# cchao0116/EasyDGL

Hardware: AMD Instinct MI355X
Metric: sequences/sec (fwd+bwd+Adam) B=512 L=100 d=128 |I|=20K (higher is better)
Workload: dtype bf16

## Files before the change

### easydgl_amd/csrc/k_encode.hip

```cpp
#include "edgl_common.h"
#include "batch_prep.h"
#include "red_batch.h"
#include "encode_scatter.h"

namespace {

using namespace enc_scatter;

struct EncP {
    const int64_t* ids; const float* ts; const void* item_tab; const float* pos_tab; const float* mark_emb;
    const uint8_t* mark_table; const float* tscale;
    int B, T, C, E, I; int64_t mask_id; float time_scale;
    float rate; const uint64_t* rng; uint32_t stream_id;
    void* x0; float* spans; uint8_t* marks;
    int dhp, dht; float sq;
};

template <typename T>
__device__ __forceinline__ void encode_fwd_block(const EncP& p, long block) {
    const int cpr = p.C >> 3;
    const long gid = block * blockDim.x + threadIdx.x;
    const long row = gid / cpr;
    if (row >= (long)p.B * p.T) return;
    const int cv = (int)(gid % cpr), c0 = cv * 8, j0 = c0 >> 1;
// ... 179 lines not shown
    __shared__ int s_lead[SROWS];
    const int SR = p.srows;
    const long rows = (long)p.B * p.T, r0 = (long)blockIdx.x * SR;
    const int tid = threadIdx.x;
    if (tid < SR) s_id[tid] = (r0 + tid < rows) ? (int)p.ids[r0 + tid] : 0;
    if (tid >= SR && tid < SROWS) s_id[tid] = -1;
    const int cpr = p.C / 4, rows_par = 256 / cpr;
    const int cv = tid % cpr, rl = tid / cpr, c0 = cv * 4;
    constexpr int MAXR = 16;
    Frag4<T> g[MAXR];
    const bool worker = tid < rows_par * cpr;
    auto item_grad = [&](long row) {
        Frag4<T> v = frag_ld<T>(reinterpret_cast<const T*>(p.dx0) + row * 3 * p.C + c0);
        if (p.add1) {
            const Frag4<T> a = frag_ld<T>(reinterpret_cast<const T*>(p.add1) + row * p.C + c0);
            const Frag4<T> b = frag_ld<T>(reinterpret_cast<const T*>(p.add2) + row * p.C + c0);
#pragma unroll
            for (int j = 0; j < 4; ++j) v.v[j] = from_f32<T>(to_f32(v.v[j]) + to_f32(a.v[j]) + to_f32(b.v[j]));
        }
        return v;
    };
#pragma unroll
    for (int k = 0; k < MAXR; ++k) g[k] = item_grad(min(r0 + rl + (long)k * rows_par, rows - 1));
    for (int i = tid; i < SR * p.C; i += 256) acc[i] = 0.f;
    __syncthreads();
    if (tid < SR) {
        const int id = s_id[tid];
        int lead = tid;
        for (int j4 = (tid >> 2); j4 >= 0; --j4) {
            const int4 v = *reinterpret_cast<const int4*>(s_id + 4 * j4);
            const int j = 4 * j4;
            if (v.w == id && j + 3 < tid) lead = j + 3;
            if (v.z == id && j + 2 < tid) lead = j + 2;
            if (v.y == id && j + 1 < tid) lead = j + 1;
            if (v.x == id && j < tid) lead = j;
        }
        s_lead[tid] = lead;
    }
    __syncthreads();
    const DropKey dk = make_dropkey(p.rng, p.stream_id, p.rate);
    const float sq = p.sq;
    if (worker) {
#pragma unroll
        for (int k = 0; k < MAXR; ++k) {
            const int r = rl + k * rows_par;
            if (r >= SR || s_id[r] == 0) continue;
            const long row = r0 + r;
            float* dst = acc + s_lead[r] * p.C + c0;
            float gv[4];
#pragma unroll
            for (int j = 0; j < 4; ++j) gv[j] = to_f32(g[k].v[j]);
            drop_apply4(dk, (uint64_t)row * 3 * p.C + c0, gv);
#pragma unroll
            for (int j = 0; j < 4; ++j) atomicAdd(dst + j, sq * gv[j]);
        }
        for (int r = rl + MAXR * rows_par; r < SR; r += rows_par) {
            if (s_id[r] == 0) continue;
            const long row = r0 + r;
            const Frag4<T> g0 = item_grad(row);
            float* dst = acc + s_lead[r] * p.C + c0;
            float gv[4];
#pragma unroll
            for (int j = 0; j < 4; ++j) gv[j] = to_f32(g0.v[j]);
            drop_apply4(dk, (uint64_t)row * 3 * p.C + c0, gv);
#pragma unroll
            for (int j = 0; j < 4; ++j) atomicAdd(dst + j, sq * gv[j]);
        }
    }
    __syncthreads();
    for (int i = tid; i < SR * p.C; i += 256) {
        const int r = i / p.C, c = i % p.C;
        if (s_lead[r] == r && s_id[r] != 0) atomicAdd(p.d_item + (long)s_id[r] * p.C + c, acc[i]);
    }
}

template <int CT>
__global__ __launch_bounds__(256) void encode_scatter_mfma_kernel(EncBwdP p, RedBatch rb) {
    constexpr int C = 16 * CT, LDG = C + 8, SR = SROWS;
    __shared__ __attribute__((aligned(16))) bf16 Gs[SR * LDG];
    __shared__ __attribute__((aligned(16))) int s_id[SR];
    __shared__ __attribute__((aligned(16))) int s_lead[SR];
    if ((int)blockIdx.x >= p.red_blk0 && (int)blockIdx.x < p.red_blk0 + rb.blocks) {
        static_assert(sizeof(Gs) >= 32 * 9 * sizeof(float4), "the reduction's scratch lives in the row image");
        reduce_rows_vec_block(rb, (int)blockIdx.x - p.red_blk0, reinterpret_cast<float4(*)[9]>(Gs));
        return;
    }
    __shared__ float s_cf[SR], s_cb[SR];
    scatter_block<CT>(p, (int)blockIdx.x - (p.red_blk0 == 0 ? rb.blocks : 0), (int)blockIdx.y, Gs, s_id, s_lead, s_cf, s_cb);
}

}

extern "C" long edgl_encode_bwd_workspace(int B, int T, int C) { (void)B; return 2L * ENC_NCHUNK * T * C; }

extern "C" int edgl_encode_fwd_ct(const int64_t* ids, const float* ts, const void* item_tab, const float* pos_tab,
                                  const float* mark_emb, const uint8_t* mark_table, const float* tscale, int B, int T,
                                  int C, int E, int I, int64_t mask_id, float time_scale, float drop_rate,
                                  const uint64_t* rng_state, uint32_t stream_id, void* x0, float* spans,
                                  uint8_t* marks, int dh_pad, int dh_true, int dtype, void* stream);
extern "C" int edgl_encode_fwd(const int64_t* ids, const float* ts, const void* item_tab, const float* pos_tab,
                               const float* mark_emb, const uint8_t* mark_table, const float* tscale, int B, int T,
                               int C, int E, int I, int64_t mask_id, float time_scale, float drop_rate,
                               const uint64_t* rng_state, uint32_t stream_id, void* x0, float* spans,
                               uint8_t* marks, int dtype, void* stream) {
    return edgl_encode_fwd_ct(ids, ts, item_tab, pos_tab, mark_emb, mark_table, tscale, B, T, C, E, I, mask_id, time_scale, drop_rate,
                              rng_state, stream_id, x0, spans, marks, 0, 0, dtype, stream);
}
extern "C" int edgl_encode_fwd_ct(const int64_t* ids, const float* ts, const void* item_tab, const float* pos_tab,
                                  const float* mark_emb, const uint8_t* mark_table, const float* tscale, int B, int T,
                                  int C, int E, int I, int64_t mask_id, float time_scale, float drop_rate,
                                  const uint64_t* rng_state, uint32_t stream_id, void* x0, float* spans,
                                  uint8_t* marks, int dh_pad, int dh_true, int dtype, void* stream) {
    EDGL_REQUIRE((dh_pad == 0 && dh_true == 0) || (dh_pad > 0 && dh_true > 0 && dh_true <= dh_pad && C % dh_pad == 0), EDGL_ERR_SHAPE,
                 "edgl_encode_fwd: padded-channel spec dh_pad=%d dh_true=%d does not fit C=%d", dh_pad, dh_true, C);
    EDGL_REQUIRE(ids && ts && item_tab && pos_tab && mark_emb && mark_table && tscale && x0 && spans && marks,
                 EDGL_ERR_NULL, "edgl_encode_fwd: null pointer");
    EDGL_REQUIRE(B > 0 && T > 0 && C > 0 && (C % 8) == 0 && E >= 1 && I > 1, EDGL_ERR_SHAPE,
                 "edgl_encode_fwd: bad shape B=%d T=%d C=%d E=%d I=%d (C must be a multiple of 8)", B, T, C, E, I);
    EDGL_REQUIRE(drop_rate == 0.f || rng_state, EDGL_ERR_NULL, "edgl_encode_fwd: dropout without rng_state");
    EncP p{ids, ts, item_tab, pos_tab, mark_emb, mark_table, tscale, B, T, C, E, I, mask_id, time_scale,
           drop_rate, rng_state, stream_id, x0, spans, marks, dh_pad, dh_true,
           sqrtf((float)(dh_pad ? C / dh_pad * dh_true : C))};
    const long total = (long)B * T * (C / 8);
    dim3 grid((unsigned)((total + 255) / 256));
    hipStream_t st = (hipStream_t)stream;
    if (dtype == EDGL_F32) hipLaunchKernelGGL((encode_fwd_kernel<float>), grid, dim3(256), 0, st, p);
    else if (dtype == EDGL_BF16) hipLaunchKernelGGL((encode_fwd_kernel<bf16>), grid, dim3(256), 0, st, p);
    else { edgl_set_error("edgl_encode_fwd: bad dtype %d", dtype); return EDGL_ERR_DTYPE; }
    EDGL_LAUNCH_CHECK();
    return EDGL_OK;
}

extern "C" int edgl_encode_fwd_prep(const int64_t* ids, const float* ts, const void* item_tab, const float* pos_tab,
                                    const float* mark_emb, const uint8_t* mark_table, const float* tscale, int B, int T,
                                    int C, int E, int I, int64_t mask_id, float time_scale, float drop_rate,
                                    const uint64_t* rng_state, uint32_t stream_id, void* x0, float* spans,
                                    uint8_t* marks, int dh_pad, int dh_true, const int64_t* labels, int M, int32_t* perm,
                                    int32_t* inv, int32_t* nvalid, int64_t* labels_c, const int64_t* masked_pos, void* tpp_desc,
                                    int dtype, void* stream) {
    EDGL_REQUIRE((dh_pad == 0 && dh_true == 0) || (dh_pad > 0 && dh_true > 0 && dh_true <= dh_pad && C % dh_pad == 0), EDGL_ERR_SHAPE,
                 "edgl_encode_fwd_prep: padded-channel spec dh_pad=%d dh_true=%d does not fit C=%d", dh_pad, dh_true, C);
    EDGL_REQUIRE(ids && ts && item_tab && pos_tab && mark_emb && mark_table && tscale && x0 && spans && marks,
                 EDGL_ERR_NULL, "edgl_encode_fwd_prep: null pointer");
    EDGL_REQUIRE(labels && perm && inv && nvalid && labels_c, EDGL_ERR_NULL, "edgl_encode_fwd_prep: null pointer (compaction)");
    EDGL_REQUIRE(B > 0 && T > 0 && C > 0 && (C % 8) == 0 && E >= 1 && I > 1 && M > 0, EDGL_ERR_SHAPE,
                 "edgl_encode_fwd_prep: bad shape B=%d T=%d C=%d E=%d I=%d M=%d (C must be a multiple of 8)", B, T, C, E, I, M);
    EDGL_REQUIRE(drop_rate == 0.f || rng_state, EDGL_ERR_NULL, "edgl_encode_fwd_prep: dropout without rng_state");
    EDGL_REQUIRE(dtype == EDGL_F32 || dtype == EDGL_BF16, EDGL_ERR_DTYPE, "edgl_encode_fwd_prep: bad dtype %d", dtype);
    if (tpp_desc) {
        EDGL_REQUIRE(masked_pos, EDGL_ERR_NULL, "edgl_encode_fwd_prep: slot data without masked positions");
        EDGL_REQUIRE(T <= 2048 && E == 16 && M <= 256, EDGL_ERR_SHAPE,
                     "edgl_encode_fwd_prep: slot data needs E = 16, M <= 256, T <= 2048 (B=%d T=%d E=%d M=%d)", B, T, E, M);
        EDGL_REQUIRE((((uintptr_t)mark_table | (uintptr_t)tpp_desc) & 15) == 0, EDGL_ERR_SHAPE,
                     "edgl_encode_fwd_prep: mark_table / tpp_desc must be 16-byte aligned");
    }
    EncP p{ids, ts, item_tab, pos_tab, mark_emb, mark_table, tscale, B, T, C, E, I, mask_id, time_scale,
           drop_rate, rng_state, stream_id, x0, spans, marks, dh_pad, dh_true,
           sqrtf((float)(dh_pad ? C / dh_pad * dh_true : C))};
    PrepP q{labels, B * M, perm, inv, nvalid, labels_c, masked_pos, ts, M, (char*)tpp_desc, 1 + (tpp_desc ? B : 0)};
    const long total = (long)B * T * (C / 8);
    dim3 grid((unsigned)((total + 255) / 256 + q.nprep));
    const size_t smem = tpp_desc ? (size_t)T * 16 + 2 * 256 * sizeof(int) : 2 * 16 * 4 * sizeof(int);
    hipStream_t st = (hipStream_t)stream;
    if (dtype == EDGL_F32) hipLaunchKernelGGL((encode_prep_kernel<float>), grid, dim3(256), smem, st, p, q);
    else hipLaunchKernelGGL((encode_prep_kernel<bf16>), grid, dim3(256), smem, st, p, q);
    EDGL_LAUNCH_CHECK();
    return EDGL_OK;
// ... 119 lines not shown
```

### easydgl_amd/csrc/k_gemm2.hip

```cpp
#include <cstdlib>

#include "edgl_common.h"
#include <cstring>
#include "encode_scatter.h"
#include "tn_group.h"

typedef __attribute__((ext_vector_type(4))) short tr_s16x4;

namespace gemm2 {

__device__ __forceinline__ uint2 tr_read(const bf16* tile, int ld, int k0, int z0, int lane) {
    const int G = lane >> 4, s = lane & 15;
    const bf16* p = tile + (k0 + 4 * G + (s >> 2)) * ld + z0 + 4 * (s & 3);
    tr_s16x4 v = __builtin_amdgcn_ds_read_tr16_b64_v4i16((__attribute__((address_space(3))) tr_s16x4*)p);
    return *reinterpret_cast<uint2*>(&v);
}
__device__ __forceinline__ bf16x8 tr_frag32(const bf16* tile, int ld, int k0, int z0, int lane) {
    bf16x8 f;
    *reinterpret_cast<uint2*>(&f) = tr_read(tile, ld, k0, z0, lane);
    *(reinterpret_cast<uint2*>(&f) + 1) = tr_read(tile, ld, k0 + 16, z0, lane);
    return f;
}

struct EpiP {
// ... 554 lines not shown
                const uint32_t keep = drop_keep4(dk, (uint64_t)row * 3 * C + c0);
#pragma unroll
                for (int j = 0; j < 4; ++j)
                    if (!((keep >> j) & 1u)) v.v[j] = from_f32<bf16>(0.f);
            }
            *reinterpret_cast<uint2*>(Os + r * G_LDO + c0) = *reinterpret_cast<const uint2*>(&v);
        }
        lds_barrier();
        scatter_onehot_sum<8>(Os, s_id, s_lead, e.d_item, C, 0, e.sq * dk.scale);
        return;
    }
    if (jn == 2) {
        if (mb0 == 0 && mt == 0 && e.d_mark_zero)
            for (int i = tid; i < e.E * C; i += G_NT) e.d_mark_zero[i] = 0.f;
        if (tid < SROWS) {
            int nm = 0;
            if (mb0 + tid < B) {
                const uint8_t* mrow = e.marks + ((long)(mb0 + tid) * T + mt) * e.E;
                for (int q = 0; q < e.E; ++q) nm += mrow[q];
            }
            s_nm[tid] = (float)nm;
        }
        lds_barrier();
    }
    double a[4] = {0., 0., 0., 0.};
#pragma unroll
    for (int k = 0; k < 16; ++k) {
        const int r = rl + 8 * k;
        if (mb0 + r < B) {
            const long row = (long)(mb0 + r) * T + mt;
            Frag4<bf16> g;
            *reinterpret_cast<uint2*>(&g) = *reinterpret_cast<const uint2*>(Os + r * G_LDO + c0);
            float v[4];
#pragma unroll
            for (int j = 0; j < 4; ++j) v[j] = to_f32(g.v[j]);
            drop_apply4(dk, (uint64_t)row * 3 * C + jn * C + c0, v);
            const double w = jn == 2 ? (double)s_nm[r] : 1.;
#pragma unroll
            for (int j = 0; j < 4; ++j) a[j] += w * (double)v[j];
        }
    }
    lds_barrier();
    double* sm = reinterpret_cast<double*>(Os);
    *reinterpret_cast<double2*>(sm + rl * C + c0) = make_double2(a[0], a[1]);
    *reinterpret_cast<double2*>(sm + rl * C + c0 + 2) = make_double2(a[2], a[3]);
    lds_barrier();
    if (tid < C) {
        double s = 0.;
#pragma unroll
        for (int i = 0; i < 8; ++i) s += sm[i * C + tid];
        float* part = jn == 1 ? e.part_pos : e.part_mk;
        part[((long)(mb0 / G_BM) * T + mt) * C + tid] = (float)s;
    }
}

template <int TM>
__device__ __forceinline__ void tn_body(const TnP& p, int bx, int by, int bz, bf16* Xs, bf16* Ys);

__global__ __launch_bounds__(G_NT, 3) void dx_encode_kernel(StripP p, DxEncP x, RedBatch rb, TnGroupP g, int tn_blocks) {
    static_assert(sizeof(StripP) + sizeof(DxEncP) + sizeof(RedBatch) + sizeof(TnGroupP) + sizeof(int) < 4096, "kernel arguments: 4 KB");
    static_assert(T_NT == G_NT && 2 * T_BR * T_LD * (int)sizeof(bf16) <= DXE_LDS, "the TN tiles run in this kernel's workgroup shape and LDS");
    extern __shared__ __attribute__((aligned(16))) char smem[];
    const int bid0 = (int)blockIdx.x;
    const int bid = bid0 - tn_blocks;
    if (bid0 < tn_blocks) {
        const int vid = xcd_virtual_id(bid0, tn_blocks, g.blk0[g.n]);
        if (vid < 0) return;
        int j = 0;
        for (int i = 1; i < g.n; ++i)
            if (vid >= g.blk0[i]) j = i;
        const int local = vid - g.blk0[j];
        const int tn = g.tiles_n[j], tk = g.tiles_k[j];
        bf16* Xs = reinterpret_cast<bf16*>(smem);
        tn_body<128>(g.job[j], local % tn, (local / tn) % tk, local / (tn * tk), Xs, Xs + T_BR * T_LD);
        return;
    }
    if (bid >= x.gemm_blocks) {
        const int e = bid - x.gemm_blocks;
        bf16* Gs = reinterpret_cast<bf16*>(smem);
        int* s_id = reinterpret_cast<int*>(Gs + G_BM * G_LDO);
        if (e < x.lab_blocks)
            enc_scatter::scatter_block<8>(x.e, x.e.lab_blk0 + e, 0, Gs, s_id, s_id + 128, reinterpret_cast<float*>(s_id + 256), reinterpret_cast<float*>(s_id + 384));
        else
            reduce_rows_vec_block(rb, e - x.lab_blocks, reinterpret_cast<float4(*)[9]>(smem));
        return;
    }
    const int vid = xcd_virtual_id(bid, x.gemm_blocks, (x.mapB + G_BM - 1) / G_BM * x.mapT * (p.N / G_BN));
    if (vid < 0) return;
    tile_nn_tile<true, false, true>(p, vid, smem, &x);
}

template <bool B_KC, bool EPI = false>
static int launch_tile_nn(const StripP& p, hipStream_t st) {
    constexpr size_t a_el = (size_t)G_BM * G_LDK, b_el = B_KC ? (size_t)G_BN * G_LDK : (size_t)G_BK * G_LDN;
    const size_t smem = std::max((EPI ? 2 : 1) * (a_el + b_el) * sizeof(bf16), (size_t)G_BM * G_LDO * sizeof(bf16));
    auto k = tile_nn_kernel<B_KC, EPI>;
    EDGL_LDS_LIMIT(k, smem, "edgl_gemm (tile)");
    const int nbm = (p.M + G_BM - 1) / G_BM, nbn = p.N / G_BN;
    hipLaunchKernelGGL(k, dim3((unsigned)xcd_grid(nbm * nbn)), dim3(G_NT), smem, st, p);
    EDGL_LAUNCH_CHECK();
    return 1;
}

template <int TM>
__device__ __forceinline__ void tn_body(const TnP& p, int bx, int by, int bz, bf16* Xs, bf16* Ys) {
    constexpr int NI = TM / 32, LDT = TM + 16, PCS = TM / 8, NLD = T_BR * PCS / T_NT;
    const int tid = threadIdx.x, lane = tid & 63, wave = tid >> 6, wm = wave >> 1, wn = wave & 1;
    const int g4 = (lane >> 4) * 4, l15 = lane & 15;
    const int kf0 = by * TM, n0 = bx * TM;
    const int r_lo = bz * p.rows_per_split, r_hi = min(p.R, r_lo + p.rows_per_split);
    f32x4 acc[NI][NI];
#pragma unroll
    for (int i = 0; i < NI; ++i)
#pragma unroll
        for (int j = 0; j < NI; ++j) acc[i][j] = f32x4{0.f, 0.f, 0.f, 0.f};
    constexpr int NCS = NI / 2;
    f32x4 acc_cs[NCS];
#pragma unroll
    for (int j = 0; j < NCS; ++j) acc_cs[j] = f32x4{0.f, 0.f, 0.f, 0.f};
    const bool do_cs = p.with_colsum && by == 0;
    bf16x8 ones;
#pragma unroll
    for (int i = 0; i < 8; ++i) ones[i] = (__bf16)1.0f;
    uint4 px[NLD], py[NLD];
    int r0_cur = 0;
    auto load = [&](int r0) {
        r0_cur = r0;
#pragma unroll
        for (int i = 0; i < NLD; ++i) {
            const int v = tid + i * T_NT, row = v / PCS, cv = v % PCS, gr = min(r0 + row, r_hi - 1);
            const int cx = min(kf0 + cv * 8, p.Kf - 8), cy = min(n0 + cv * 8, p.N - 8);
            px[i] = *reinterpret_cast<const uint4*>(p.X + (long)gr * p.ldx + cx);
            py[i] = *reinterpret_cast<const uint4*>(p.Y + (long)gr * p.ldy + cy);
        }
    };
    auto store = [&]() {
#pragma unroll
        for (int i = 0; i < NLD; ++i) {
            const int v = tid + i * T_NT, row = v / PCS, cv = v % PCS;
            const bool ok = r0_cur + row < r_hi;
            *reinterpret_cast<uint4*>(Xs + row * LDT + cv * 8) = ok ? px[i] : make_uint4(0, 0, 0, 0);
            *reinterpret_cast<uint4*>(Ys + row * LDT + cv * 8) = ok ? py[i] : make_uint4(0, 0, 0, 0);
        }
    };
    const int nstep = (r_hi - r_lo + T_BR - 1) / T_BR;
    if (nstep > 0) { load(r_lo); store(); }
    __syncthreads();
    for (int st = 0; st < nstep; ++st) {
        const bool more = st + 1 < nstep;
        if (more) load(r_lo + (st + 1) * T_BR);
#pragma unroll
        for (int rb = 0; rb < T_BR / 32; ++rb) {
            bf16x8 af[NI], bf_[NI];
#pragma unroll
            for (int i = 0; i < NI; ++i) af[i] = tr_frag32(Xs, LDT, rb * 32, wm * (TM / 2) + i * 16, lane);
#pragma unroll
            for (int j = 0; j < NI; ++j) bf_[j] = tr_frag32(Ys, LDT, rb * 32, wn * (TM / 2) + j * 16, lane);
#pragma unroll
            for (int i = 0; i < NI; ++i)
#pragma unroll
                for (int j = 0; j < NI; ++j) acc[i][j] = __builtin_amdgcn_mfma_f32_16x16x32_bf16(af[i], bf_[j], acc[i][j], 0, 0, 0);
            if (do_cs) {
                if (wm) {
#pragma unroll
                    for (int j = 0; j < NCS; ++j) acc_cs[j] = __builtin_amdgcn_mfma_f32_16x16x32_bf16(ones, bf_[NCS + j], acc_cs[j], 0, 0, 0);
                } else {
#pragma unroll
// ... 307 lines not shown
```

### easydgl_amd/csrc/k_reduce.hip

```cpp
#include "edgl_common.h"
#include "red_batch.h"

namespace {

__global__ __launch_bounds__(256) void reduce_rows_kernel(const float* part, int P, int N, long ld, float* out, int accumulate) {
    __shared__ float sm[8][33];
    const int tx = threadIdx.x & 31, ty = threadIdx.x >> 5;
    const int n = blockIdx.x * 32 + tx;
    float a0 = 0.f, a1 = 0.f, a2 = 0.f, a3 = 0.f;
    if (n < N) {
        int p = ty;
        for (; p + 24 < P; p += 32) {
            a0 += part[(long)p * ld + n];
            a1 += part[(long)(p + 8) * ld + n];
            a2 += part[(long)(p + 16) * ld + n];
            a3 += part[(long)(p + 24) * ld + n];
        }
        for (; p < P; p += 8) a0 += part[(long)p * ld + n];
    }
    sm[ty][tx] = (a0 + a1) + (a2 + a3);
    __syncthreads();
    if (ty == 0 && n < N) {
        float s = 0.f;
#pragma unroll
        for (int i = 0; i < 8; ++i) s += sm[i][tx];
        out[n] = accumulate ? out[n] + s : s;
    }
}

}

static inline int red_blocks_scalar(const RedJob& j) { return (j.N + 31) / 32; }
static inline int red_blocks_vec(const RedJob& j) { return j.P <= RED_COL_P && !j.f64 ? (j.N + 1023) / 1024 : (j.N + 31) / 32; }
static inline bool red_job_vec(const RedJob& j) {
    return (j.N & 3) == 0 && (j.ld & 3) == 0 && (((uintptr_t)j.part | (uintptr_t)j.out) & 15) == 0;
}
static void red_assign_blocks(RedBatch& b, bool vec) {
    int blocks = 0;
    for (int i = 0; i < b.n; ++i) {
        b.j[i].blk0 = blocks;
        blocks += vec ? red_blocks_vec(b.j[i]) : red_blocks_scalar(b.j[i]);
    }
    b.blocks = blocks;
}
thread_local bool g_red_defer = false;
thread_local RedBatch g_red_batch = {};
thread_local int g_red_ride = 0;

template <int RL>
__global__ __launch_bounds__(32 * RL) void reduce_rows_multi_kernel(RedBatch b) {
    __shared__ float sm[RL][33];
    int ji = 0;
    for (int i = 1; i < b.n; ++i)
        if ((int)blockIdx.x >= b.j[i].blk0) ji = i;
    const RedJob& jb = b.j[ji];
    const float* part = jb.part;
    const int P = jb.P, N = jb.N;
    const long ld = jb.ld;
    const int tx = threadIdx.x & 31, ty = threadIdx.x >> 5;
    const int n = ((int)blockIdx.x - jb.blk0) * 32 + tx;
    float a0 = 0.f, a1 = 0.f, a2 = 0.f, a3 = 0.f;
    if (n < N) {
        int p = ty;
        for (; p + 3 * RL < P; p += 4 * RL) {
            a0 += part[(long)p * ld + n];
            a1 += part[(long)(p + RL) * ld + n];
            a2 += part[(long)(p + 2 * RL) * ld + n];
            a3 += part[(long)(p + 3 * RL) * ld + n];
        }
        for (; p < P; p += RL) a0 += part[(long)p * ld + n];
    }
    sm[ty][tx] = (a0 + a1) + (a2 + a3);
    __syncthreads();
    if (ty == 0 && n < N) {
        float s = 0.f;
#pragma unroll
        for (int i = 0; i < RL; ++i) s += sm[i][tx];
        jb.out[n] = s;
    }
}

__global__ __launch_bounds__(256) void reduce_rows_multi_vec_kernel(RedBatch b) {
    __shared__ float4 sm[32][9];
    reduce_rows_vec_block(b, (int)blockIdx.x, sm);
}

int edgl_reduce_flush_impl(hipStream_t st) {
    if (g_red_batch.n == 0) return EDGL_OK;
    int maxp = 0;
    bool vec = true;
    for (int i = 0; i < g_red_batch.n; ++i) {
        const RedJob& j = g_red_batch.j[i];
        maxp = std::max(maxp, j.P);
        vec = vec && red_job_vec(j);
    }
    red_assign_blocks(g_red_batch, vec);
    if (vec) hipLaunchKernelGGL(reduce_rows_multi_vec_kernel, dim3(g_red_batch.blocks), dim3(256), 0, st, g_red_batch);
    else if (maxp > 1024) hipLaunchKernelGGL(reduce_rows_multi_kernel<32>, dim3(g_red_batch.blocks), dim3(1024), 0, st, g_red_batch);
    else hipLaunchKernelGGL(reduce_rows_multi_kernel<8>, dim3(g_red_batch.blocks), dim3(256), 0, st, g_red_batch);
    g_red_batch.n = 0;
    g_red_batch.blocks = 0;
    EDGL_LAUNCH_CHECK();
    return EDGL_OK;
}

int edgl_reduce_rows(const float* part, int P, int N, long ld, float* out, int accumulate, hipStream_t st) {
    if (g_red_defer && !accumulate) {
        if (g_red_batch.n == RED_MAX_JOBS) {
            const int rc = edgl_reduce_flush_impl(st);
            if (rc) return rc;
        }
        RedJob& j = g_red_batch.j[g_red_batch.n++];
        j.part = part; j.out = out; j.ld = ld; j.P = P; j.N = N; j.blk0 = g_red_batch.blocks; j.f64 = 0;
        g_red_batch.blocks += (N + 31) / 32;
        return EDGL_OK;
    }
    if (g_red_defer) {
        const int rc = edgl_reduce_flush_impl(st);
        if (rc) return rc;
    }
    hipLaunchKernelGGL(reduce_rows_kernel, dim3((N + 31) / 32), dim3(256), 0, st, part, P, N, ld, out, accumulate);
    EDGL_LAUNCH_CHECK();
    return EDGL_OK;
}

int edgl_reduce_ride_take(const RedJob* own, int nown, const float* lo0, const float* hi0, const float* lo1, const float* hi1,
                          RedBatch* out, int* first_blocks, hipStream_t st) {
    if (!g_red_defer || !g_red_ride) return 0;
    auto rides = [&](const RedJob& j) {
        const float* o0 = j.out;
        const float* o1 = j.out + j.N;
        return red_job_vec(j) && !(o0 < hi0 && lo0 < o1) && !(o0 < hi1 && lo1 < o1);
    };
    for (int i = 0; i < g_red_batch.n; ++i)
        if (!rides(g_red_batch.j[i])) return 0;
    for (int i = 0; i < nown; ++i)
        if (!rides(own[i])) return 0;
    if (g_red_batch.n + nown > RED_MAX_JOBS) {
        const int rc = edgl_reduce_flush_impl(st);
        if (rc) return rc;
    }
    for (int i = 0; i < nown; ++i) g_red_batch.j[g_red_batch.n++] = own[i];
    red_assign_blocks(g_red_batch, true);
    const int blocks = g_red_batch.blocks;
    *out = g_red_batch;
    *first_blocks = g_red_ride == 1;
    g_red_batch.n = 0;
    g_red_batch.blocks = 0;
    return blocks;
}

int edgl_reduce_rows_now(const RedJob* jobs, int n, hipStream_t st) {
    if (n <= 0) return EDGL_OK;
    bool vec = n <= RED_MAX_JOBS;
    for (int i = 0; i < n && vec; ++i) vec = red_job_vec(jobs[i]);
    if (!vec) {
        for (int i = 0; i < n; ++i) {
            const int rc = edgl_reduce_rows(jobs[i].part, jobs[i].P, jobs[i].N, jobs[i].ld, jobs[i].out, 0, st);
            if (rc) return rc;
        }
        return EDGL_OK;
    }
    RedBatch b;
    b.n = n;
    for (int i = 0; i < n; ++i) b.j[i] = jobs[i];
    red_assign_blocks(b, true);
    hipLaunchKernelGGL(reduce_rows_multi_vec_kernel, dim3(b.blocks), dim3(256), 0, st, b);
    EDGL_LAUNCH_CHECK();
    return EDGL_OK;
}

int edgl_reduce_rows_f64(const float* part, int P, int N, long ld, float* out, hipStream_t st) {
    const RedJob j{part, out, ld, P, N, g_red_batch.blocks, 1};
    if (!red_job_vec(j)) return edgl_reduce_rows(part, P, N, ld, out, 0, st);
    if (!g_red_defer) return edgl_reduce_rows_now(&j, 1, st);
    if (g_red_batch.n == RED_MAX_JOBS) {
        const int rc = edgl_reduce_flush_impl(st);
        if (rc) return rc;
    }
    g_red_batch.j[g_red_batch.n] = j;
    g_red_batch.j[g_red_batch.n++].blk0 = g_red_batch.blocks;
    g_red_batch.blocks += (N + 31) / 32;
    return EDGL_OK;
}

extern "C" int edgl_reduce_ride(int on) {
    EDGL_REQUIRE(on >= 0 && on <= 2, EDGL_ERR_SHAPE, "edgl_reduce_ride: on = %d (0: off, 1: in front of the scatter's workgroups, 2: behind)", on);
    g_red_ride = on;
    return EDGL_OK;
}

extern "C" int edgl_reduce_partials(const float* part, int P, int N, long ld, float* out, int accumulate, void* stream) {
    EDGL_REQUIRE(part && out, EDGL_ERR_NULL, "edgl_reduce_partials: null pointer");
    EDGL_REQUIRE(P > 0 && N > 0 && ld >= N, EDGL_ERR_SHAPE, "edgl_reduce_partials: bad shape P=%d N=%d ld=%ld", P, N, ld);
    return edgl_reduce_rows(part, P, N, ld, out, accumulate, (hipStream_t)stream);
}

extern "C" int edgl_reduce_defer(int on, void* stream) {
    if (on <= 0) g_red_ride = 0;
    if (on < 0) {
        g_red_batch.n = 0;
        g_red_batch.blocks = 0;
        g_red_defer = false;
        return EDGL_OK;
    }
    if (!on && g_red_defer) {
        const int rc = edgl_reduce_flush_impl((hipStream_t)stream);
        if (rc) return rc;
    }
    g_red_defer = on != 0;
    return EDGL_OK;
}

extern "C" int edgl_reduce_flush(void* stream) { return edgl_reduce_flush_impl((hipStream_t)stream); }
```

### easydgl_amd/csrc/k_score.hip

```cpp
#include <cstdlib>
#include <mutex>
#include <unordered_map>

#include "edgl_common.h"
#include "score_plan.h"
#include "score_strip.h"

namespace {

constexpr int SNT = 512;

template <typename T, int CT>
struct ScoreCfg {
    static constexpr bool BF = sizeof(T) == 2;
    static constexpr bool STD = CT <= 8 || (BF && CT == 16);
    static constexpr int IX = STD ? 2 : 1;
    static constexpr int ZB = STD ? 128 : ((BF || CT == 16) ? 64 : 32);
    static constexpr int NWB = (!BF && CT == 32) ? 4 : 8;
    static constexpr int CO = (BF && CT >= 16) ? CT / 2 : CT;
};
struct RtCfg { int ix, zb, nwb; };
inline RtCfg rt_cfg(int C, size_t esize) {
    const int ct = C / 16;
    const bool bf = esize == 2, stdc = ct <= 8 || (bf && ct == 16);
// ... 663 lines not shown
    TO* out = reinterpret_cast<TO*>(j.out);
    if constexpr (sizeof(TO) == 4) {
        if (((j.lo | j.hi | j.n | j.zero_first) & 3) == 0 && ((uintptr_t)j.slabs & 15) == 0 && ((uintptr_t)out & 15) == 0) {
            for (long i = j.lo + (bid * blockDim.x + threadIdx.x) * 4; i < j.hi; i += nblk * blockDim.x * 4) {
                float4 a = make_float4(0.f, 0.f, 0.f, 0.f);
                for (int s0 = 0; s0 < nslab; s0 += 4) {
                    float4 x[4];
#pragma unroll
                    for (int k = 0; k < 4; ++k) x[k] = *reinterpret_cast<const float4*>(j.slabs + (long)min(s0 + k, nslab - 1) * j.n + i);
#pragma unroll
                    for (int k = 0; k < 4; ++k) {
                        const float w = s0 + k < nslab ? 1.f : 0.f;
                        a.x = s0 + k < nslab ? a.x + x[k].x : a.x; a.y = s0 + k < nslab ? a.y + x[k].y : a.y;
                        a.z = s0 + k < nslab ? a.z + x[k].z : a.z; a.w = s0 + k < nslab ? a.w + x[k].w : a.w;
                        (void)w;
                    }
                }
                const bool z = i < j.zero_first;
                *reinterpret_cast<float4*>(out + i) = z ? make_float4(0.f, 0.f, 0.f, 0.f) : make_float4(a.x * gs, a.y * gs, a.z * gs, a.w * gs);
            }
            return;
        }
    }
    for (long i = j.lo + bid * blockDim.x + threadIdx.x; i < j.hi; i += nblk * blockDim.x) {
        float a = 0.f;
        for (int s = 0; s < nslab; ++s) a += j.slabs[(long)s * j.n + i];
        out[i] = from_f32<TO>(i < j.zero_first ? 0.f : a * gs);
    }
}

template <typename TO>
__global__ void slab_reduce_rows_kernel(const float* slabs, const int32_t* nvalid, int R, int C, int xb, int zb, int G, int ztotal,
                                        const float* gscale, TO* out) {
    const float gs = gscale ? gscale[0] : 1.0f;
    const int Reff = nvalid ? min(R, nvalid[0]) : R;
    const DevPlan dp = dev_plan(Reff, xb, G, ztotal, zb);
    const long stride = (long)dp.nx * xb * C, nval = (long)Reff * C, n = (long)R * C;
    for (long i = (long)blockIdx.x * blockDim.x + threadIdx.x; i < n; i += (long)gridDim.x * blockDim.x) {
        float a = 0.f;
        if (i < nval)
            for (int s = 0; s < dp.nchunk; ++s) a += slabs[(long)s * stride + i];
        out[i] = from_f32<TO>(a * gs);
    }
}

template <bool S16>
__device__ __forceinline__ float4 ld_slab4(const float* slabs, long off) {
    if constexpr (S16) {
        const uint2 u = *reinterpret_cast<const uint2*>(reinterpret_cast<const bf16*>(slabs) + off);
        return make_float4(__uint_as_float(u.x << 16), __uint_as_float(u.x & 0xffff0000u), __uint_as_float(u.y << 16), __uint_as_float(u.y & 0xffff0000u));
    } else {
        return *reinterpret_cast<const float4*>(slabs + off);
    }
}

template <typename TO, int LPR, bool S16 = false>
__global__ __launch_bounds__(256) void flash_finish_lse_kernel(const float* slabs, const float* part, const TO* rows, const TO* table,
                                                               const float* out_bias, const int64_t* labels, const int32_t* nvalid,
                                                               const int32_t* wtotal, int R, int xb, int zb, int G, int ztotal,
                                                               const float* gscale, float* row_lse, float* lab_out, float* coef_out,
                                                               TO* out, float* ce_part) {
    constexpr int C = 4 * LPR, MAXCH = 16;
    __shared__ float ce_red[8];
    float ce_num = 0.f;
    const float gs = gscale ? gscale[0] : 1.0f;
    const int Reff = nvalid ? min(R, nvalid[0]) : R;
    const float W = (float)(wtotal ? wtotal[0] : Reff) + 1e-5f;
    const DevPlan dp = dev_plan(max(Reff, 1), xb, G, ztotal, zb);
    const long stride = (long)dp.nx * xb * C;
    const int nch = dp.nchunk;
    const int nrow_blk = 256 / LPR;
    for (long r0 = (long)blockIdx.x * nrow_blk; r0 < R; r0 += (long)gridDim.x * nrow_blk) {
        const int r = (int)min(r0 + threadIdx.x / LPR, (long)R - 1), c = (threadIdx.x % LPR) * 4, rc = min(r, max(Reff - 1, 0));
        const bool live = r0 + threadIdx.x / LPR < R;
        if (r0 >= Reff) {
            if (live) {
                if (c == 0) { row_lse[r] = 0.f; lab_out[r] = labels[r] == 0 ? -1000.0f : 0.f; coef_out[r] = 0.f; }
                if constexpr (sizeof(TO) == 2) *reinterpret_cast<uint2*>(out + (long)r * C + c) = make_uint2(0u, 0u);
                else *reinterpret_cast<float4*>(out + (long)r * C + c) = make_float4(0.f, 0.f, 0.f, 0.f);
            }
            continue;
        }
        int64_t lab = labels[r];
        asm volatile("" : "+v"(lab));
        const int64_t labc = lab > 0 ? lab : 0;
        float ob = out_bias[max(labc, (int64_t)1) - 1];
        float xr[4], tb[4];
        if constexpr (sizeof(TO) == 2) {
            const Frag4<TO> fx = frag_ld<TO>(rows + (long)r * C + c), ft = frag_ld<TO>(table + labc * C + c);
#pragma unroll
            for (int q = 0; q < 4; ++q) { xr[q] = to_f32(fx.v[q]); tb[q] = to_f32(ft.v[q]); }
        } else {
            const float4 fx = *reinterpret_cast<const float4*>(rows + (long)r * C + c), ft = *reinterpret_cast<const float4*>(table + labc * C + c);
            xr[0] = fx.x; xr[1] = fx.y; xr[2] = fx.z; xr[3] = fx.w; tb[0] = ft.x; tb[1] = ft.y; tb[2] = ft.z; tb[3] = ft.w;
        }
        float mx = -INFINITY;
        float4 sl0[MAXCH];
        float pm0[MAXCH], ps0[MAXCH];
#pragma unroll
        for (int s = 0; s < MAXCH; ++s) {
            const int sc = min(s, nch - 1);
            sl0[s] = ld_slab4<S16>(slabs, (long)sc * stride + (long)rc * C + c);
            pm0[s] = part[((long)rc * nch + sc) * 2];
            ps0[s] = part[((long)rc * nch + sc) * 2 + 1];
        }
#pragma unroll
        for (int s = 0; s < MAXCH; ++s) mx = s < nch ? fmaxf(mx, pm0[s]) : mx;
        for (int s0 = MAXCH; s0 < nch; s0 += MAXCH) {
            float pm[MAXCH];
#pragma unroll
            for (int s = 0; s < MAXCH; ++s) pm[s] = part[((long)rc * nch + min(s0 + s, nch - 1)) * 2];
#pragma unroll
            for (int s = 0; s < MAXCH; ++s) mx = s0 + s < nch ? fmaxf(mx, pm[s]) : mx;
        }
        float sm = 0.f, acc[4] = {0.f, 0.f, 0.f, 0.f};
#pragma unroll
        for (int s = 0; s < MAXCH; ++s) {
            const float e = (s < nch && pm0[s] > -INFINITY) ? __expf(pm0[s] - mx) : 0.f;
            sm = fmaf(ps0[s], e, sm);
            acc[0] = fmaf(sl0[s].x, e, acc[0]); acc[1] = fmaf(sl0[s].y, e, acc[1]);
            acc[2] = fmaf(sl0[s].z, e, acc[2]); acc[3] = fmaf(sl0[s].w, e, acc[3]);
        }
        for (int s0 = MAXCH; s0 < nch; s0 += MAXCH) {
            float4 sl[MAXCH];
            float pm[MAXCH], ps[MAXCH];
#pragma unroll
            for (int s = 0; s < MAXCH; ++s) {
                const int sc = min(s0 + s, nch - 1);
                sl[s] = ld_slab4<S16>(slabs, (long)sc * stride + (long)rc * C + c);
                pm[s] = part[((long)rc * nch + sc) * 2];
                ps[s] = part[((long)rc * nch + sc) * 2 + 1];
            }
#pragma unroll
            for (int s = 0; s < MAXCH; ++s) {
                const float e = (s0 + s < nch && pm[s] > -INFINITY) ? __expf(pm[s] - mx) : 0.f;
                sm = fmaf(ps[s], e, sm);
                acc[0] = fmaf(sl[s].x, e, acc[0]); acc[1] = fmaf(sl[s].y, e, acc[1]);
                acc[2] = fmaf(sl[s].z, e, acc[2]); acc[3] = fmaf(sl[s].w, e, acc[3]);
            }
        }
        asm volatile("" : "+v"(ob));
        const float lse = r < Reff ? mx + __logf(sm) : 0.f;
        const float inv_sm = (r < Reff && sm > 0.f) ? 1.0f / sm : 0.f;
        float a = (xr[0] * tb[0] + xr[1] * tb[1]) + (xr[2] * tb[2] + xr[3] * tb[3]);
#pragma unroll
        for (int o = LPR / 2; o > 0; o >>= 1) a += __shfl_xor(a, o, 64);
        const float ll = lab == 0 ? -1000.0f : a + ob;
        const float v = __expf(ll - lse);
        const float cf = (r < Reff && lab != 0) ? (1.f / W) * (v / (v + 1e-5f)) : 0.f;
        if (live && c == 0) {
            row_lse[r] = lse; lab_out[r] = ll; coef_out[r] = cf;
            ce_num += (r < Reff && lab != 0) ? -__logf(v + 1e-5f) : 0.f;
        }
#pragma unroll
        for (int q = 0; q < 4; ++q) acc[q] *= inv_sm;
        float o4[4];
#pragma unroll
        for (int q = 0; q < 4; ++q) o4[q] = cf != 0.f ? gs * cf * (acc[q] - tb[q]) : 0.f;
        if (live) {
            if constexpr (sizeof(TO) == 2) { const Frag4<TO> f = frag_from_acc<TO>(f32x4{o4[0], o4[1], o4[2], o4[3]}); *reinterpret_cast<uint2*>(out + (long)r * C + c) = *reinterpret_cast<const uint2*>(&f); }
            else *reinterpret_cast<float4*>(out + (long)r * C + c) = make_float4(o4[0], o4[1], o4[2], o4[3]);
        }
    }
    if (ce_part) {
        ce_num = block_sum(ce_num, ce_red);
        if (threadIdx.x == 0) {
            ce_part[blockIdx.x] = ce_num;
            if (blockIdx.x == 0) ce_part[gridDim.x] = (float)Reff;
        }
    }
}

template <typename TO, int LPR, bool S16 = false, int CPL = 8>
__global__ __launch_bounds__(256) void flash_finish_lse_wide_kernel(const float* slabs, const float* part, const TO* rows, const TO* table,
                                                               const float* out_bias, const int64_t* labels, const int32_t* nvalid,
                                                               const int32_t* wtotal, int R, int xb, int zb, int G, int ztotal,
                                                               const float* gscale, float* row_lse, float* lab_out, float* coef_out,
                                                               TO* out, float* ce_part) {
    constexpr int C = CPL * LPR, MAXCH = CPL == 4 ? 16 : 8, NQ = CPL / 4;
    __shared__ float ce_red[8];
    float ce_num = 0.f;
    const float gs = gscale ? gscale[0] : 1.0f;
    const int Reff = nvalid ? min(R, nvalid[0]) : R;
    const float W = (float)(wtotal ? wtotal[0] : Reff) + 1e-5f;
    const DevPlan dp = dev_plan(max(Reff, 1), xb, G, ztotal, zb);
    const long stride = (long)dp.nx * xb * C;
    const int nch = dp.nchunk;
    const int nrow_blk = 256 / LPR;
    for (long r0 = (long)blockIdx.x * nrow_blk; r0 < R; r0 += (long)gridDim.x * nrow_blk) {
        const int r = (int)min(r0 + threadIdx.x / LPR, (long)R - 1), c = (threadIdx.x % LPR) * CPL, rc = min(r, max(Reff - 1, 0));
        const bool live = r0 + threadIdx.x / LPR < R;
        if (r0 >= Reff) {
            if (live) {
                if (c == 0) { row_lse[r] = 0.f; lab_out[r] = labels[r] == 0 ? -1000.0f : 0.f; coef_out[r] = 0.f; }
#pragma unroll
                for (int h = 0; h < NQ; ++h) {
                    if constexpr (sizeof(TO) == 2) *reinterpret_cast<uint2*>(out + (long)r * C + c + 4 * h) = make_uint2(0u, 0u);
                    else *reinterpret_cast<float4*>(out + (long)r * C + c + 4 * h) = make_float4(0.f, 0.f, 0.f, 0.f);
                }
            }
            continue;
        }
        int64_t lab = labels[r];
        asm volatile("" : "+v"(lab));
        const int64_t labc = lab > 0 ? lab : 0;
        float ob = out_bias[max(labc, (int64_t)1) - 1];
        float xr[CPL], tb[CPL];
#pragma unroll
        for (int h = 0; h < NQ; ++h) {
            if constexpr (sizeof(TO) == 2) {
                const Frag4<TO> fx = frag_ld<TO>(rows + (long)r * C + c + 4 * h), ft = frag_ld<TO>(table + labc * C + c + 4 * h);
#pragma unroll
                for (int q = 0; q < 4; ++q) { xr[4 * h + q] = to_f32(fx.v[q]); tb[4 * h + q] = to_f32(ft.v[q]); }
            } else {
                const float4 fx = *reinterpret_cast<const float4*>(rows + (long)r * C + c + 4 * h), ft = *reinterpret_cast<const float4*>(table + labc * C + c + 4 * h);
                xr[4 * h] = fx.x; xr[4 * h + 1] = fx.y; xr[4 * h + 2] = fx.z; xr[4 * h + 3] = fx.w;
                tb[4 * h] = ft.x; tb[4 * h + 1] = ft.y; tb[4 * h + 2] = ft.z; tb[4 * h + 3] = ft.w;
            }
        }
        float mx = -INFINITY;
        float4 sl0[MAXCH][NQ];
        float pm0[MAXCH], ps0[MAXCH];
#pragma unroll
        for (int s = 0; s < MAXCH; ++s) {
// ... 621 lines not shown
```

### easydgl_amd/csrc/red_batch.h

```cpp
#pragma once
#include "edgl_common.h"

constexpr int RED_MAX_JOBS = 24;
constexpr int RED_COL_P = 32;
struct RedJob { const float* part; float* out; long ld; int P, N, blk0, f64; };
struct RedBatch { RedJob j[RED_MAX_JOBS]; int n, blocks; };

int edgl_reduce_ride_take(const RedJob* own, int nown, const float* lo0, const float* hi0, const float* lo1, const float* hi1,
                          RedBatch* out, int* first_blocks, hipStream_t st);

int edgl_reduce_rows_now(const RedJob* jobs, int n, hipStream_t st);
int edgl_reduce_rows_f64(const float* part, int P, int N, long ld, float* out, hipStream_t st);

__device__ __forceinline__ void reduce_rows_vec_block(const RedBatch& b, int bid, float4 (*sm)[9]) {
    int ji = 0;
    for (int i = 1; i < b.n; ++i)
        if (bid >= b.j[i].blk0) ji = i;
    const RedJob& jb = b.j[ji];
    const int P = jb.P, N = jb.N;
    const long ld = jb.ld;
    if (jb.f64) {
        const int tx = threadIdx.x & 7, ty = threadIdx.x >> 3;
        const int n = (bid - jb.blk0) * 32 + 4 * tx;
        double a[4] = {0., 0., 0., 0.};
        if (n < N)
            for (int p = ty; p < P; p += 32) {
                const float4 v = *reinterpret_cast<const float4*>(jb.part + n + (long)p * ld);
                a[0] += v.x; a[1] += v.y; a[2] += v.z; a[3] += v.w;
            }
        double2 (*sd)[9] = reinterpret_cast<double2(*)[9]>(sm);
#pragma unroll
        for (int h = 0; h < 2; ++h) {
            sd[ty][tx] = make_double2(a[2 * h], a[2 * h + 1]);
            __syncthreads();
            if (ty < 2 && n < N) {
                double s = 0.;
#pragma unroll
                for (int i = 0; i < 32; ++i) s += ty == 0 ? sd[i][tx].x : sd[i][tx].y;
                jb.out[n + 2 * h + ty] = (float)s;
            }
            __syncthreads();
        }
        return;
    }
    if (P <= RED_COL_P) {
        const int n = ((bid - jb.blk0) * 256 + (int)threadIdx.x) * 4;
        if (n >= N) return;
        const float* base = jb.part + n;
        float4 acc = make_float4(0.f, 0.f, 0.f, 0.f);
        int p0 = 0;
        for (; p0 + 8 <= P; p0 += 8) {
            float4 v[8];
#pragma unroll
            for (int u = 0; u < 8; ++u) v[u] = *reinterpret_cast<const float4*>(base + (long)(p0 + u) * ld);
#pragma unroll
            for (int u = 0; u < 8; ++u) { acc.x += v[u].x; acc.y += v[u].y; acc.z += v[u].z; acc.w += v[u].w; }
        }
        for (; p0 < P; ++p0) {
            const float4 v = *reinterpret_cast<const float4*>(base + (long)p0 * ld);
            acc.x += v.x; acc.y += v.y; acc.z += v.z; acc.w += v.w;
        }
        *reinterpret_cast<float4*>(jb.out + n) = acc;
        return;
    }
    const int tx = threadIdx.x & 7, ty = threadIdx.x >> 3;
    const int n = (bid - jb.blk0) * 32 + 4 * tx;
    float4 acc = make_float4(0.f, 0.f, 0.f, 0.f);
    if (n < N) {
        const float* base = jb.part + n;
        int p = ty;
        for (; p + 7 * 32 < P; p += 8 * 32) {
            float4 v[8];
#pragma unroll
            for (int u = 0; u < 8; ++u) v[u] = *reinterpret_cast<const float4*>(base + (long)(p + 32 * u) * ld);
#pragma unroll
            for (int u = 0; u < 8; ++u) { acc.x += v[u].x; acc.y += v[u].y; acc.z += v[u].z; acc.w += v[u].w; }
        }
        for (; p < P; p += 32) {
            const float4 v = *reinterpret_cast<const float4*>(base + (long)p * ld);
            acc.x += v.x; acc.y += v.y; acc.z += v.z; acc.w += v.w;
        }
    }
    sm[ty][tx] = acc;
    __syncthreads();
    if (ty < 4 && n < N) {
        float s = 0.f;
#pragma unroll
        for (int i = 0; i < 32; ++i) {
            const float4 v = sm[i][tx];
            s += ty == 0 ? v.x : (ty == 1 ? v.y : (ty == 2 ? v.z : v.w));
        }
        jb.out[n + ty] = s;
    }
}
```

Measured before the change: 742,100.

## Template row reduction on column width and load depth; hoist score row loads

Reworks the column-partial reduction into a template on column width and load-batch depth. Standalone reduce launches use one float per thread with 32 loads in flight, which gives more blocks. Reductions that ride inside other kernels keep float4 columns with 8 in flight. Tail handling now clamps and masks loads instead of using scalar remainder loops, f64 jobs also take the column path, and in the score kernel the row and label-table fragment loads are issued earlier so their latency overlaps the partial-max loads. The changes add register pressure and more block-count bookkeeping, and the gain depends on how the compiler schedules the pinned loads.

```diff
diff --git a/easydgl_amd/csrc/k_encode.hip b/easydgl_amd/csrc/k_encode.hip
--- a/easydgl_amd/csrc/k_encode.hip
+++ b/easydgl_amd/csrc/k_encode.hip
@@ -285,7 +285,7 @@
     __shared__ __attribute__((aligned(16))) int s_lead[SR];
     if ((int)blockIdx.x >= p.red_blk0 && (int)blockIdx.x < p.red_blk0 + rb.blocks) {
         static_assert(sizeof(Gs) >= 32 * 9 * sizeof(float4), "the reduction's scratch lives in the row image");
-        reduce_rows_vec_block(rb, (int)blockIdx.x - p.red_blk0, reinterpret_cast<float4(*)[9]>(Gs));
+        reduce_rows_vec_block<RED_CW_RIDE, RED_DC_RIDE>(rb, (int)blockIdx.x - p.red_blk0, reinterpret_cast<float4(*)[9]>(Gs));
         return;
     }
     __shared__ float s_cf[SR], s_cb[SR];
diff --git a/easydgl_amd/csrc/k_gemm2.hip b/easydgl_amd/csrc/k_gemm2.hip
--- a/easydgl_amd/csrc/k_gemm2.hip
+++ b/easydgl_amd/csrc/k_gemm2.hip
@@ -660,7 +660,7 @@
         if (e < x.lab_blocks)
             enc_scatter::scatter_block<8>(x.e, x.e.lab_blk0 + e, 0, Gs, s_id, s_id + 128, reinterpret_cast<float*>(s_id + 256), reinterpret_cast<float*>(s_id + 384));
         else
-            reduce_rows_vec_block(rb, e - x.lab_blocks, reinterpret_cast<float4(*)[9]>(smem));
+            reduce_rows_vec_block<RED_CW_RIDE, RED_DC_RIDE>(rb, e - x.lab_blocks, reinterpret_cast<float4(*)[9]>(smem));
         return;
     }
     const int vid = xcd_virtual_id(bid, x.gemm_blocks, (x.mapB + G_BM - 1) / G_BM * x.mapT * (p.N / G_BN));
diff --git a/easydgl_amd/csrc/k_reduce.hip b/easydgl_amd/csrc/k_reduce.hip
--- a/easydgl_amd/csrc/k_reduce.hip
+++ b/easydgl_amd/csrc/k_reduce.hip
@@ -31,15 +31,15 @@
 }
 
 static inline int red_blocks_scalar(const RedJob& j) { return (j.N + 31) / 32; }
-static inline int red_blocks_vec(const RedJob& j) { return j.P <= RED_COL_P && !j.f64 ? (j.N + 1023) / 1024 : (j.N + 31) / 32; }
+static inline int red_blocks_vec(const RedJob& j, int cw) { return j.P <= RED_COL_P ? (j.N + red_col_span(cw) - 1) / red_col_span(cw) : (j.N + 31) / 32; }
 static inline bool red_job_vec(const RedJob& j) {
     return (j.N & 3) == 0 && (j.ld & 3) == 0 && (((uintptr_t)j.part | (uintptr_t)j.out) & 15) == 0;
 }
-static void red_assign_blocks(RedBatch& b, bool vec) {
+static void red_assign_blocks(RedBatch& b, bool vec, int cw = RED_CW_OWN) {
     int blocks = 0;
     for (int i = 0; i < b.n; ++i) {
         b.j[i].blk0 = blocks;
-        blocks += vec ? red_blocks_vec(b.j[i]) : red_blocks_scalar(b.j[i]);
+        blocks += vec ? red_blocks_vec(b.j[i], cw) : red_blocks_scalar(b.j[i]);
     }
     b.blocks = blocks;
 }
@@ -82,7 +82,7 @@
 
 __global__ __launch_bounds__(256) void reduce_rows_multi_vec_kernel(RedBatch b) {
     __shared__ float4 sm[32][9];
-    reduce_rows_vec_block(b, (int)blockIdx.x, sm);
+    reduce_rows_vec_block<RED_CW_OWN, RED_DC_OWN>(b, (int)blockIdx.x, sm);
 }
 
 int edgl_reduce_flush_impl(hipStream_t st) {
@@ -141,7 +141,7 @@
         if (rc) return rc;
     }
     for (int i = 0; i < nown; ++i) g_red_batch.j[g_red_batch.n++] = own[i];
-    red_assign_blocks(g_red_batch, true);
+    red_assign_blocks(g_red_batch, true, RED_CW_RIDE);
     const int blocks = g_red_batch.blocks;
     *out = g_red_batch;
     *first_blocks = g_red_ride == 1;
diff --git a/easydgl_amd/csrc/k_score.hip b/easydgl_amd/csrc/k_score.hip
--- a/easydgl_amd/csrc/k_score.hip
+++ b/easydgl_amd/csrc/k_score.hip
@@ -769,18 +769,12 @@
             continue;
         }
         int64_t lab = labels[r];
-        asm volatile("" : "+v"(lab));
-        const int64_t labc = lab > 0 ? lab : 0;
-        float ob = out_bias[max(labc, (int64_t)1) - 1];
         float xr[4], tb[4];
-        if constexpr (sizeof(TO) == 2) {
-            const Frag4<TO> fx = frag_ld<TO>(rows + (long)r * C + c), ft = frag_ld<TO>(table + labc * C + c);
-#pragma unroll
-            for (int q = 0; q < 4; ++q) { xr[q] = to_f32(fx.v[q]); tb[q] = to_f32(ft.v[q]); }
-        } else {
-            const float4 fx = *reinterpret_cast<const float4*>(rows + (long)r * C + c), ft = *reinterpret_cast<const float4*>(table + labc * C + c);
-            xr[0] = fx.x; xr[1] = fx.y; xr[2] = fx.z; xr[3] = fx.w; tb[0] = ft.x; tb[1] = ft.y; tb[2] = ft.z; tb[3] = ft.w;
-        }
+        Frag4<TO> fx16;
+        float4 fx32;
+        if constexpr (sizeof(TO) == 2) fx16 = frag_ld<TO>(rows + (long)r * C + c);
+        else fx32 = *reinterpret_cast<const float4*>(rows + (long)r * C + c);
+        EDGL_PIN();
         float mx = -INFINITY;
         float4 sl0[MAXCH];
         float pm0[MAXCH], ps0[MAXCH];
@@ -791,6 +785,15 @@
             pm0[s] = part[((long)rc * nch + sc) * 2];
             ps0[s] = part[((long)rc * nch + sc) * 2 + 1];
         }
+        EDGL_PIN();
+        asm volatile("" : "+v"(lab));
+        const int64_t labc = lab > 0 ? lab : 0;
+        float ob = out_bias[max(labc, (int64_t)1) - 1];
+        Frag4<TO> ft16;
+        float4 ft32;
+        if constexpr (sizeof(TO) == 2) ft16 = frag_ld<TO>(table + labc * C + c);
+        else ft32 = *reinterpret_cast<const float4*>(table + labc * C + c);
+        EDGL_PIN();
 #pragma unroll
         for (int s = 0; s < MAXCH; ++s) mx = s < nch ? fmaxf(mx, pm0[s]) : mx;
         for (int s0 = MAXCH; s0 < nch; s0 += MAXCH) {
@@ -827,6 +830,14 @@
             }
         }
         asm volatile("" : "+v"(ob));
+        if constexpr (sizeof(TO) == 2) {
+            touch_regs(ft16);
+#pragma unroll
+            for (int q = 0; q < 4; ++q) { xr[q] = to_f32(fx16.v[q]); tb[q] = to_f32(ft16.v[q]); }
+        } else {
+            touch_regs(ft32);
+            xr[0] = fx32.x; xr[1] = fx32.y; xr[2] = fx32.z; xr[3] = fx32.w; tb[0] = ft32.x; tb[1] = ft32.y; tb[2] = ft32.z; tb[3] = ft32.w;
+        }
         const float lse = r < Reff ? mx + __logf(sm) : 0.f;
         const float inv_sm = (r < Reff && sm > 0.f) ? 1.0f / sm : 0.f;
         float a = (xr[0] * tb[0] + xr[1] * tb[1]) + (xr[2] * tb[2] + xr[3] * tb[3]);
diff --git a/easydgl_amd/csrc/red_batch.h b/easydgl_amd/csrc/red_batch.h
--- a/easydgl_amd/csrc/red_batch.h
+++ b/easydgl_amd/csrc/red_batch.h
@@ -12,6 +12,54 @@
 int edgl_reduce_rows_now(const RedJob* jobs, int n, hipStream_t st);
 int edgl_reduce_rows_f64(const float* part, int P, int N, long ld, float* out, hipStream_t st);
 
+constexpr int RED_CW_RIDE = 4, RED_DC_RIDE = 8;
+constexpr int RED_CW_OWN = 1, RED_DC_OWN = 32;
+constexpr int RED_DR = 8;
+__host__ __device__ constexpr int red_col_span(int cw) { return 256 * cw; }
+
+template <int CW> struct RedVec;
+template <> struct RedVec<1> { using type = float; };
+template <> struct RedVec<4> { using type = float4; };
+__device__ __forceinline__ float red_comp(const float& v, int) { return v; }
+__device__ __forceinline__ float red_comp(const float4& v, int q) { return q == 0 ? v.x : (q == 1 ? v.y : (q == 2 ? v.z : v.w)); }
+
+template <typename V, int D>
+__device__ __forceinline__ void red_load_batch(V (&v)[D], const float* base, long ld, int p0, int step, int P) {
+    static_assert(D % 8 == 0 && D >= 8, "batches are made of groups of eight loads");
+#pragma unroll
+    for (int g = 0; g < D; g += 8) {
+        if (p0 + g * step < P) {
+#pragma unroll
+            for (int u = g; u < g + 8; ++u) v[u] = *reinterpret_cast<const V*>(base + (long)min(p0 + u * step, P - 1) * ld);
+        }
+    }
+}
+
+template <typename ACC, int CW, int DC>
+__device__ __forceinline__ void reduce_rows_col(const RedJob& jb, int blk) {
+    using V = typename RedVec<CW>::type;
+    const int n = (blk * 256 + (int)threadIdx.x) * CW;
+    if (n >= jb.N) return;
+    const int P = jb.P;
+    const float* base = jb.part + n;
+    ACC a[CW];
+#pragma unroll
+    for (int q = 0; q < CW; ++q) a[q] = (ACC)0;
+    for (int p0 = 0; p0 < P; p0 += DC) {
+        V v[DC];
+        red_load_batch<V, DC>(v, base, jb.ld, p0, 1, P);
+#pragma unroll
+        for (int u = 0; u < DC; ++u)
+            if (p0 + u < P) {
+#pragma unroll
+                for (int q = 0; q < CW; ++q) a[q] += red_comp(v[u], q);
+            }
+    }
+    if constexpr (CW == 4) *reinterpret_cast<float4*>(jb.out + n) = make_float4((float)a[0], (float)a[1], (float)a[2], (float)a[3]);
+    else jb.out[n] = (float)a[0];
+}
+
+template <int CW, int DC>
 __device__ __forceinline__ void reduce_rows_vec_block(const RedBatch& b, int bid, float4 (*sm)[9]) {
     int ji = 0;
     for (int i = 1; i < b.n; ++i)
@@ -19,14 +67,22 @@
     const RedJob& jb = b.j[ji];
     const int P = jb.P, N = jb.N;
     const long ld = jb.ld;
+    if (P <= RED_COL_P) {
+        if (jb.f64) reduce_rows_col<double, CW, DC>(jb, bid - jb.blk0);
+        else reduce_rows_col<float, CW, DC>(jb, bid - jb.blk0);
+        return;
+    }
+    const int tx = threadIdx.x & 7, ty = threadIdx.x >> 3;
+    const int n = (bid - jb.blk0) * 32 + 4 * tx;
     if (jb.f64) {
-        const int tx = threadIdx.x & 7, ty = threadIdx.x >> 3;
-        const int n = (bid - jb.blk0) * 32 + 4 * tx;
         double a[4] = {0., 0., 0., 0.};
         if (n < N)
-            for (int p = ty; p < P; p += 32) {
-                const float4 v = *reinterpret_cast<const float4*>(jb.part + n + (long)p * ld);
-                a[0] += v.x; a[1] += v.y; a[2] += v.z; a[3] += v.w;
+            for (int p = ty; p < P; p += 32 * RED_DR) {
+                float4 v[RED_DR];
+                red_load_batch<float4, RED_DR>(v, jb.part + n, ld, p, 32, P);
+#pragma unroll
+                for (int u = 0; u < RED_DR; ++u)
+                    if (p + 32 * u < P) { a[0] += v[u].x; a[1] += v[u].y; a[2] += v[u].z; a[3] += v[u].w; }
             }
         double2 (*sd)[9] = reinterpret_cast<double2(*)[9]>(sm);
 #pragma unroll
@@ -43,44 +99,15 @@
         }
         return;
     }
-    if (P <= RED_COL_P) {
-        const int n = ((bid - jb.blk0) * 256 + (int)threadIdx.x) * 4;
-        if (n >= N) return;
-        const float* base = jb.part + n;
-        float4 acc = make_float4(0.f, 0.f, 0.f, 0.f);
-        int p0 = 0;
-        for (; p0 + 8 <= P; p0 += 8) {
-            float4 v[8];
+    float4 acc = make_float4(0.f, 0.f, 0.f, 0.f);
+    if (n < N)
+        for (int p = ty; p < P; p += 32 * RED_DR) {
+            float4 v[RED_DR];
+            red_load_batch<float4, RED_DR>(v, jb.part + n, ld, p, 32, P);
 #pragma unroll
-            for (int u = 0; u < 8; ++u) v[u] = *reinterpret_cast<const float4*>(base + (long)(p0 + u) * ld);
-#pragma unroll
-            for (int u = 0; u < 8; ++u) { acc.x += v[u].x; acc.y += v[u].y; acc.z += v[u].z; acc.w += v[u].w; }
+            for (int u = 0; u < RED_DR; ++u)
+                if (p + 32 * u < P) { acc.x += v[u].x; acc.y += v[u].y; acc.z += v[u].z; acc.w += v[u].w; }
         }
-        for (; p0 < P; ++p0) {
-            const float4 v = *reinterpret_cast<const float4*>(base + (long)p0 * ld);
-            acc.x += v.x; acc.y += v.y; acc.z += v.z; acc.w += v.w;
-        }
-        *reinterpret_cast<float4*>(jb.out + n) = acc;
-        return;
-    }
-    const int tx = threadIdx.x & 7, ty = threadIdx.x >> 3;
-    const int n = (bid - jb.blk0) * 32 + 4 * tx;
-    float4 acc = make_float4(0.f, 0.f, 0.f, 0.f);
-    if (n < N) {
-        const float* base = jb.part + n;
-        int p = ty;
-        for (; p + 7 * 32 < P; p += 8 * 32) {
-            float4 v[8];
-#pragma unroll
-            for (int u = 0; u < 8; ++u) v[u] = *reinterpret_cast<const float4*>(base + (long)(p + 32 * u) * ld);
-#pragma unroll
-            for (int u = 0; u < 8; ++u) { acc.x += v[u].x; acc.y += v[u].y; acc.z += v[u].z; acc.w += v[u].w; }
-        }
-        for (; p < P; p += 32) {
-            const float4 v = *reinterpret_cast<const float4*>(base + (long)p * ld);
-            acc.x += v.x; acc.y += v.y; acc.z += v.z; acc.w += v.w;
-        }
-    }
     sm[ty][tx] = acc;
     __syncthreads();
     if (ty < 4 && n < N) {
```

New measurement: 743,600, median of 6. Within noise of the previous version (+0.2%).
